# microsoft/VidTok

Measured on NVIDIA H100. Metric: frames/sec encode+decode, kl_causal_488 17x256x256, higher is better.
Workload: dtype bf16

## Files before the change

### vidtok_b200/csrc/conv_tc.cu

```cuda
#include <cuda.h>

#include <cstdio>
#include <cstdlib>
#include <cstring>
#include <string>
#include <type_traits>

#include "common.cuh"
#include "kernels.h"
#include "tc_ptx.cuh"

namespace vt {

namespace {

thread_local std::string g_tc_err;

struct TcParams {
  int B, To, Ho, Wo, Co, Ti;
  int BW, BH, BT;
  int tilesW, tilesH, tilesT;
  int num_n_tiles, BN;
  long long num_tiles;
  int kt, kh, kw, Ci, num_kc;
// ... 14 lines not shown
  int Co_real;
  int w_batched;
  int ln_mode, ln_silu;
  const float* ln_gamma;
  const float* ln_beta;
  void* out2;
  int res_mma;
  int halo, hP, a_stages;
  uint32_t halo_bytes;
  int split, a_lo, b_lo, o_lo;
  float acc_scale;
  int kparts;
  int reg_mode, reg_zc, reg_sample;
  const float* reg_noise;
  float* reg_z;
  int* reg_idx;
  double* reg_kl;
  FsqConst reg_fsq;
  uint32_t misc_off;
};

struct TcMaps {
  CUtensorMap a[4];
  CUtensorMap c;
  CUtensorMap b;
  CUtensorMap r;
  CUtensorMap e;
};

constexpr int kConsumerWarps = 8;
constexpr int kProducerWarp = kConsumerWarps;
constexpr int kThreads = (kConsumerWarps + 4) * 32;
constexpr int kABytes = 128 * 128;

using namespace tcx;

struct TileCoord {
  int b, t0, h0, w0, n0;
};
__device__ __forceinline__ TileCoord decode_tile(const TcParams& p, long long tile) {
  TileCoord c;
  const int nt = (int)(tile % p.num_n_tiles);
  long long m = tile / p.num_n_tiles;
  const int tw = (int)(m % p.tilesW); m /= p.tilesW;
  const int th = (int)(m % p.tilesH); m /= p.tilesH;
  const int tt = (int)(m % p.tilesT);
  c.b = (int)(m / p.tilesT);
  c.t0 = tt * p.BT; c.h0 = th * p.BH; c.w0 = tw * p.BW; c.n0 = nt * p.BN;
  return c;
}
__device__ __forceinline__ bool tap_time(const TcParams& p, const TileCoord& tc, int a, int& tv, bool& from_cache) {
  tv = (tc.t0 + p.to_off) * p.st + a - p.pt;
  from_cache = false;
  if (tv + p.BT <= 0) {
    if (p.t_mode == 0) return false;
    if (p.t_mode == 1) { tv = 0; return true; }
    from_cache = true;
    tv = p.cacheT + tv;
    return true;
  }
  return true;
}

__device__ __forceinline__ float quad_sum(float v) {
  v += __shfl_xor_sync(0xffffffffu, v, 1);
  v += __shfl_xor_sync(0xffffffffu, v, 2);
  return v;
}

template <int BN, bool kSplit>
__global__ void __launch_bounds__(kThreads, 1)
conv_tc_kernel(const __grid_constant__ TcMaps maps, const TcParams p) {
  extern __shared__ uint8_t smem_raw[];
  const uint32_t smem_base = (smem_u32(smem_raw) + 1023u) & ~1023u;
  uint8_t* smem_gen = smem_raw + (smem_base - smem_u32(smem_raw));
  const int warp = threadIdx.x >> 5, lane = threadIdx.x & 31;
  const uint32_t a_bytes = kABytes;
  constexpr uint32_t b_bytes = (uint32_t)BN * 128u;
  constexpr uint32_t kPl = kSplit ? 2u : 1u;
  const uint32_t stage_bytes = kPl * (p.halo ? b_bytes : a_bytes + b_bytes);
  const uint32_t win_bytes = kPl * p.halo_bytes;
  const uint32_t ring_base = smem_base + (p.halo ? (uint32_t)p.a_stages * win_bytes : 0u);
  const uint32_t bar_base = ring_base + p.stages * stage_bytes;
  auto full_bar = [&](int s) { return bar_base + 8u * s; };
  auto empty_bar = [&](int s) { return bar_base + 8u * (p.stages + s); };
  auto fullA_bar = [&](int s) { return bar_base + 8u * (2 * p.stages + s); };
  auto emptyA_bar = [&](int s) { return bar_base + 8u * (2 * p.stages + p.a_stages + s); };
  float* sbias = reinterpret_cast<float*>(smem_gen + p.misc_off);
  float* rowbuf = sbias + 2 * 768;

  if (threadIdx.x == 0) {
    for (int s = 0; s < p.stages; ++s) {
      mbar_init(full_bar(s), 1);
      mbar_init(empty_bar(s), kConsumerWarps);
    }
    for (int s = 0; s < p.a_stages; ++s) {
      mbar_init(fullA_bar(s), 1);
      mbar_init(emptyA_bar(s), kConsumerWarps);
    }
    asm volatile("fence.mbarrier_init.release.cluster;" ::: "memory");
  }
  __syncthreads();

  const int nsp = p.kh * p.kw;
  const int num_kc = p.num_kc, nstages = p.stages;
  const bool halo = p.halo != 0;
  const int res_steps = p.res_mma ? BN / 64 : 0;

  if (warp >= kProducerWarp) {
    asm volatile("setmaxnreg.dec.sync.aligned.u32 40;" ::: "memory");
    if (warp != kProducerWarp) return;
    const bool el = elect_one();
    if (el) {
      prefetch_tmap(&maps.a[0]);
      prefetch_tmap(&maps.b);
      if (p.sp == 2) { prefetch_tmap(&maps.a[1]); prefetch_tmap(&maps.a[2]); prefetch_tmap(&maps.a[3]); }
      if (p.t_mode == 2) prefetch_tmap(&maps.c);
      if (p.res_mma) { prefetch_tmap(&maps.r); prefetch_tmap(&maps.e); }
    }
    int stage = 0, sA = 0;
    uint32_t phase = 0, phA = 0;
    auto acquire = [&](uint32_t bytes) {
      mbar_wait(empty_bar(stage), phase ^ 1u);
      if (el) mbar_expect_tx(full_bar(stage), bytes);
    };
    auto advance = [&]() { if (++stage == nstages) { stage = 0; phase ^= 1u; } };
    auto load_b_planes = [&](uint32_t dst, const CUtensorMap* m, int kcol, int n, int wb_) {
      tma_load_3d(dst, m, full_bar(stage), kcol, n, wb_);
      if constexpr (kSplit) tma_load_3d(dst + b_bytes, m, full_bar(stage), p.b_lo + kcol, n, wb_);
    };
    auto load_window = [&](const CUtensorMap* m, int c0, int lo_off, int cw, int ch, int ct, int cb) {
// ... 46 lines not shown
                  const uint32_t sa = smem_base + stage * stage_bytes;
                  tma_load_5d(sa, mapA, full_bar(stage), kc * 64, cw, ch, tv, tc.b);
                  if constexpr (kSplit) tma_load_5d(sa + a_bytes, mapA, full_bar(stage), p.a_lo + kc * 64, cw, ch, tv, tc.b);
                  load_b_planes(sa + kPl * a_bytes, &maps.b, kcol + kc * 64, tc.n0, wb);
                }
                advance();
              }
            }
          }
        }
      }
      for (int g = 0; g < res_steps; ++g) {
        if (halo) {
          load_window(&maps.r, tc.n0 + g * 64, p.o_lo, tc.w0 - p.pw, tc.h0 - p.ph, tc.t0, tc.b);
          acquire(b_bytes);
          if (el) tma_load_3d(ring_base + stage * stage_bytes, &maps.e, full_bar(stage), g * 64, 0, 0);
        } else {
          acquire(kPl * a_bytes + b_bytes);
          if (el) {
            const uint32_t sa = smem_base + stage * stage_bytes;
            tma_load_5d(sa, &maps.r, full_bar(stage), tc.n0 + g * 64, tc.w0, tc.h0, tc.t0, tc.b);
            if constexpr (kSplit) tma_load_5d(sa + a_bytes, &maps.r, full_bar(stage), p.o_lo + tc.n0 + g * 64, tc.w0, tc.h0, tc.t0, tc.b);
            tma_load_3d(sa + kPl * a_bytes, &maps.e, full_bar(stage), g * 64, 0, 0);
          }
        }
        advance();
      }
    }
    return;
  }

  asm volatile("setmaxnreg.inc.sync.aligned.u32 232;" ::: "memory");
  constexpr int R = BN / 2;
  constexpr bool kSum = kSplit && BN <= 128;
  const int g = warp >> 2, wq = warp & 3;
  const bool leader = lane == 0;
  const uint32_t hi_b = desc_hi(1024u);
  const uint32_t hi_a = halo ? desc_hi((uint32_t)p.hP * 128u) : hi_b;
  const uint32_t a_row_off = halo ? (uint32_t)(8 * g) * (uint32_t)p.hP * 128u : (uint32_t)g * 64u * 128u;
  const uint32_t a_pl = halo ? p.halo_bytes : a_bytes;
  const uint32_t b_addr0 = halo ? ring_base : smem_base + kPl * a_bytes;
  float acc[R];
  float sum[kSum ? R : 1];
  int stage = 0, sA = 0, sR = 0;
  uint32_t phase = 0, phA = 0;
  int pend_stage = -1;
  bool pend_win = false;
  auto release = [&]() {
    if (leader) {
      if (pend_stage >= 0) mbar_arrive(empty_bar(pend_stage));
      if (pend_win) mbar_arrive(emptyA_bar(sR));
    }
    if (pend_win && ++sR == p.a_stages) sR = 0;
    pend_stage = -1;
    pend_win = false;
  };
  auto kstep = [&](bool a_from_stage, uint32_t a_addr, uint32_t scale, bool res, bool last_of_window) {
    mbar_wait(full_bar(stage), phase);
    if (a_from_stage) a_addr = smem_base + stage * stage_bytes + a_row_off;
    const uint32_t b_addr = b_addr0 + stage * stage_bytes;
    const uint32_t al = desc_lo(a_addr), bl = desc_lo(b_addr);
    wgmma_fence();
#pragma unroll
    for (uint32_t j = 0; j < 4u; ++j) {
      const uint64_t ah = desc(al + 2u * j, hi_a), bh = desc(bl + 2u * j, hi_b);
      wgmma_k16<BN, kSplit>(acc, ah, bh, j == 0 ? scale : 1u);
      if constexpr (kSplit) {
        wgmma_k16<BN, kSplit>(acc, desc(al + (a_pl >> 4) + 2u * j, hi_a), bh, 1u);
        if (!res) wgmma_k16<BN, kSplit>(acc, ah, desc(bl + (b_bytes >> 4) + 2u * j, hi_b), 1u);
      }
    }
    wgmma_commit();
    wgmma_wait<1>();
    release();
    pend_stage = stage;
    pend_win = last_of_window;
    if (++stage == nstages) { stage = 0; phase ^= 1u; }
  };

  const int rbase = 64 * g + 16 * wq + (lane >> 2);
  const int cq = 2 * (lane & 3);
  const bool res_direct = (p.res_mode == 1 && !p.res_mma);
  const bool store_a = (p.ln_mode != 1);
  const float inv_n = 1.0f / (float)BN;
  int last_n0 = -1;
  uint32_t cbuf = 1;

  for (long long tile = blockIdx.x; tile < p.num_tiles; tile += gridDim.x) {
    const TileCoord tc = decode_tile(p, tile);
    uint32_t G = 0xFFFFFFFFu;
    if constexpr (kSum) {
      if (p.kparts > 1) {
        uint32_t nk = 0;
        for (int a = 0; a < p.kt; ++a) {
          int tv_;
          bool fc_;
          if (tap_time(p, tc, a, tv_, fc_)) nk += (uint32_t)(nsp * num_kc);
        }
        nk += (uint32_t)res_steps;
        G = (nk + (uint32_t)p.kparts - 1u) / (uint32_t)p.kparts;
      }
#pragma unroll
      for (int i = 0; i < R; ++i) sum[i] = 0.f;
    }
    uint32_t ks = 0, accum = 0;
    auto step = [&](bool a_from_stage, uint32_t a_addr, bool res, bool last_of_window) {
      if constexpr (kSum) {
        if (ks > 0 && ks % G == 0) {
          wgmma_wait<0>();
          acc_fence(acc);
          release();
#pragma unroll
          for (int i = 0; i < R; ++i) sum[i] += acc[i];
          accum = 0;
        }
      }
      kstep(a_from_stage, a_addr, accum, res, last_of_window);
      accum = 1;
      ++ks;
    };
    for (int a = 0; a < p.kt; ++a) {
      int tv;
      bool from_cache;
      if (!tap_time(p, tc, a, tv, from_cache)) continue;
      if (halo) {
        for (int kc = 0; kc < num_kc; ++kc) {
          mbar_wait(fullA_bar(sA), phA);
          const uint32_t win = smem_base + (uint32_t)sA * win_bytes + a_row_off;
          for (int bb = 0; bb < p.kh; ++bb)
            for (int c = 0; c < p.kw; ++c)
              step(false, win + (uint32_t)(bb * p.hP + c) * 128u, false, bb == p.kh - 1 && c == p.kw - 1);
          if (++sA == p.a_stages) { sA = 0; phA ^= 1u; }
        }
      } else {
        for (int s = nsp * num_kc; s > 0; --s) step(true, 0u, false, false);
      }
    }
    for (int gr = 0; gr < res_steps; ++gr) {
      if (halo) {
        mbar_wait(fullA_bar(sA), phA);
        step(false, smem_base + (uint32_t)sA * win_bytes + a_row_off + (uint32_t)(p.ph * p.hP + p.pw) * 128u, true, true);
        if (++sA == p.a_stages) { sA = 0; phA ^= 1u; }
      } else {
        step(true, 0u, true, false);
      }
    }
    wgmma_wait<0>();
    acc_fence(acc);
    release();
    if constexpr (kSum) {
#pragma unroll
      for (int i = 0; i < R; ++i) acc[i] += sum[i];
    }

    if (tc.n0 != last_n0) {
      last_n0 = tc.n0;
      cbuf ^= 1u;
      float* b_ = sbias + cbuf * 768;
      for (int i = threadIdx.x; i < BN; i += kConsumerWarps * 32) {
        b_[i] = (p.bias && tc.n0 + i < p.Co_real) ? p.bias[tc.n0 + i] : 0.f;
        if (p.ln_mode) { const float sc = (p.ln_silu && !kSplit) ? 0.5f : 1.0f; b_[256 + i] = sc * p.ln_gamma[tc.n0 + i]; b_[512 + i] = sc * p.ln_beta[tc.n0 + i]; }
      }
      asm volatile("bar.sync 1, %0;" ::"n"(kConsumerWarps * 32) : "memory");
    }
    const float* bias_s = sbias + cbuf * 768;
    const float* gamma_s = bias_s + 256;
    const float* beta_s = bias_s + 512;

    bool valid[2];
    long long ooff[2];
    const bf16* r0[2];
    const bf16* r1[2];
    const bf16* r2[2];
    auto row_geom = [&](int row, int& t, int& h, int& w) {
      const int dw = halo ? (row & 7) : row % p.BW;
      const int dh = halo ? (row >> 3) : (row / p.BW) % p.BH;
      const int dt = halo ? 0 : row / (p.BW * p.BH);
      t = tc.t0 + dt; h = tc.h0 + dh; w = tc.w0 + dw;
      return (t < p.To) && (h < p.Ho) && (w < p.Wo);
    };
#pragma unroll
    for (int r = 0; r < 2; ++r) {
      int t, h, w;
      valid[r] = row_geom(rbase + 8 * r, t, h, w);
      ooff[r] = (long long)tc.b * p.osB + (long long)t * p.osT + (long long)h * p.osH + (long long)w * p.osW;
      r0[r] = r1[r] = r2[r] = nullptr;
      if (valid[r] && res_direct) {
        r0[r] = p.res + (long long)tc.b * p.rsB + (long long)t * p.rsT + (long long)h * p.rsH + (long long)w * p.rsW + tc.n0;
      } else if (valid[r] && p.res_mode == 3) {
        const long long sp = (long long)tc.b * p.rsB + (long long)h * p.rsH + (long long)w * p.rsW + tc.n0;
        const int ta = 2 * t - 1 + p.res_pool_off, tb = ta + 1, tcn = ta + 2;
        if (ta >= 0) r0[r] = p.res + sp + (long long)ta * p.rsT;
        else if (p.res_t_mode == 1) r0[r] = p.res + sp;
        else if (p.res_t_mode == 2) r0[r] = p.res_cache + (((long long)tc.b * p.Ho + h) * p.Wo + w) * (long long)p.Co * (kSplit ? 2 : 1) + tc.n0;
        if (tb < p.resT) r1[r] = p.res + sp + (long long)tb * p.rsT;
        if (tcn < p.resT) r2[r] = p.res + sp + (long long)tcn * p.rsT;
      }
    }
    auto res_pair = [&](const bf16* rp, int c, float& x0, float& x1) {
      const uint32_t hw = *reinterpret_cast<const uint32_t*>(rp + c);
      if constexpr (kSplit) {
        const uint32_t lw = *reinterpret_cast<const uint32_t*>(rp + p.o_lo + c);
        x0 = f16_lo(hw) + f16_lo(lw);
        x1 = f16_hi(hw) + f16_hi(lw);
      } else {
        x0 = bf16_lo(hw);
        x1 = bf16_hi(hw);
      }
    };
#pragma unroll
    for (int j = 0; j < BN / 8; ++j) {
      const int c = 8 * j + cq;
#pragma unroll
      for (int e = 0; e < 4; ++e) {
        float f = kSplit ? fmaf(acc[4 * j + e], p.acc_scale, bias_s[c + (e & 1)]) : acc[4 * j + e] + bias_s[c + (e & 1)];
        if (p.rb != 1.0f) f *= p.rb;
        acc[4 * j + e] = f;
      }
#pragma unroll
      for (int r = 0; r < 2; ++r) {
        if (!valid[r]) continue;
        if (res_direct) {
          float x0, x1;
          res_pair(r0[r], c, x0, x1);
          acc[4 * j + 2 * r] = fmaf(p.ra, x0, acc[4 * j + 2 * r]);
          acc[4 * j + 2 * r + 1] = fmaf(p.ra, x1, acc[4 * j + 2 * r + 1]);
        } else if (p.res_mode == 3) {
          float s0 = 0.f, s1 = 0.f, x0, x1;
          if (r0[r]) { res_pair(r0[r], c, x0, x1); s0 += x0; s1 += x1; }
          if (r1[r]) { res_pair(r1[r], c, x0, x1); s0 += x0; s1 += x1; }
          if (r2[r]) { res_pair(r2[r], c, x0, x1); s0 += x0; s1 += x1; }
          const float s3 = p.ra * (1.0f / 3.0f);
          acc[4 * j + 2 * r] = fmaf(s3, s0, acc[4 * j + 2 * r]);
          acc[4 * j + 2 * r + 1] = fmaf(s3, s1, acc[4 * j + 2 * r + 1]);
        }
      }
    }

    if (p.out_f32) {
      if (p.out) {
#pragma unroll
        for (int r = 0; r < 2; ++r) {
          if (!valid[r]) continue;
          float* of = reinterpret_cast<float*>(p.out) + ooff[r];
#pragma unroll
          for (int j = 0; j < BN / 8; ++j)
#pragma unroll
            for (int e = 0; e < 2; ++e) {
              const int n = tc.n0 + 8 * j + cq + e;
              if (n < p.Co_real) of[(long long)n * p.osC] = acc[4 * j + 2 * r + e];
            }
        }
      }
      if (p.reg_mode) {
        if constexpr (BN == 32) {
#pragma unroll
          for (int j = 0; j < 4; ++j)
#pragma unroll
            for (int e = 0; e < 4; ++e) rowbuf[(rbase + 8 * (e >> 1)) * 33 + 8 * j + cq + (e & 1)] = acc[4 * j + e];
          asm volatile("bar.sync 2, %0;" ::"n"(kConsumerWarps * 32) : "memory");
          if (threadIdx.x < 128) {
            const int row = threadIdx.x;
            float f[32];
#pragma unroll
            for (int c = 0; c < 32; ++c) f[c] = rowbuf[row * 33 + c];
            int t, h, w;
            const bool ok = row_geom(row, t, h, w);
            const long long plane = p.osC;
            const long long pos = (long long)t * p.osT + (long long)h * p.osH + (long long)w * p.osW;
            if (p.reg_mode == 1) {
              float part = 0.f;
              auto kl_row = [&](auto ZC) {
                constexpr int zc = decltype(ZC)::value;
                const long long zb = (long long)tc.b * zc * plane + pos;
#pragma unroll
                for (int c = 0; c < zc; ++c) {
                  float zv;
                  part += kl_sample_one(f[c], f[zc + c], p.reg_sample ? p.reg_noise[zb + c * plane] : 0.f, p.reg_sample, zv);
                  p.reg_z[zb + c * plane] = zv;
                }
              };
              if (ok) {
                if (p.reg_zc == 4) kl_row(std::integral_constant<int, 4>());
                else if (p.reg_zc == 8) kl_row(std::integral_constant<int, 8>());
                else kl_row(std::integral_constant<int, 16>());
              }
              double dsum = (double)part;
#pragma unroll
              for (int o = 16; o > 0; o >>= 1) dsum += __shfl_xor_sync(0xffffffffu, dsum, o);
              if (lane == 0) atomicAdd(p.reg_kl, dsum);
            } else if (ok) {
              const long long zb = (long long)tc.b * p.reg_zc * plane + pos;
              float idx = 0.f;
#pragma unroll
              for (int c = 0; c < VT_MAX_FSQ; ++c)
                if (c < p.reg_zc) p.reg_z[zb + c * plane] = fsq_code(p.reg_fsq, c, f[c], idx);
              if (p.reg_idx) p.reg_idx[(long long)tc.b * plane + pos] = (int)idx;
            }
          }
          asm volatile("bar.sync 2, %0;" ::"n"(kConsumerWarps * 32) : "memory");
        }
      }
      continue;
    }

    auto put = [&](void* optr, int r, int c, float y0, float y1) {
      bf16* o = reinterpret_cast<bf16*>(optr) + ooff[r] + tc.n0 + c;
      if constexpr (kSplit) {
        const uint32_t hw = pack_f16x2(y0, y1);
        *reinterpret_cast<uint32_t*>(o) = hw;
        *reinterpret_cast<uint32_t*>(o + p.o_lo) = pack_f16x2(y0 - f16_lo(hw), y1 - f16_hi(hw));
      } else {
        *reinterpret_cast<uint32_t*>(o) = pack_bf16x2(y0, y1);
      }
    };
    if constexpr (kSplit) {
      if (store_a) {
#pragma unroll
        for (int r = 0; r < 2; ++r)
          if (valid[r])
#pragma unroll
            for (int j = 0; j < BN / 8; ++j) put(p.out, r, 8 * j + cq, acc[4 * j + 2 * r], acc[4 * j + 2 * r + 1]);
      }
      if (p.ln_mode) {
        void* nout = p.ln_mode == 1 ? p.out : p.out2;
#pragma unroll
        for (int r = 0; r < 2; ++r) {
          float s = 0.f;
#pragma unroll
          for (int j = 0; j < BN / 8; ++j) s += acc[4 * j + 2 * r] + acc[4 * j + 2 * r + 1];
          const float mean = quad_sum(s) * inv_n;
          float q = 0.f;
#pragma unroll
          for (int j = 0; j < BN / 8; ++j) {
            const float d0 = acc[4 * j + 2 * r] - mean, d1 = acc[4 * j + 2 * r + 1] - mean;
            q = fmaf(d0, d0, q);
            q = fmaf(d1, d1, q);
          }
          const float rstd = 1.0f / sqrtf(quad_sum(q) * inv_n + 1e-6f);
          if (!valid[r]) continue;
#pragma unroll
          for (int j = 0; j < BN / 8; ++j) {
            const int c = 8 * j + cq;
            float y0 = (acc[4 * j + 2 * r] - mean) * rstd * gamma_s[c] + beta_s[c];
            float y1 = (acc[4 * j + 2 * r + 1] - mean) * rstd * gamma_s[c + 1] + beta_s[c + 1];
            if (p.ln_silu) { y0 = silu_tc(y0); y1 = silu_tc(y1); }
            put(nout, r, c, y0, y1);
          }
        }
      }
    } else {
#pragma unroll
      for (int r = 0; r < 2; ++r) {
        float s = 0.f, q = 0.f;
#pragma unroll
        for (int j = 0; j < BN / 8; ++j) {
          const float f0 = acc[4 * j + 2 * r], f1 = acc[4 * j + 2 * r + 1];
          s += f0 + f1;
          q = fmaf(f0, f0, q);
          q = fmaf(f1, f1, q);
          const uint32_t kp = pack_bf16x2(f0, f1);
          if (store_a && valid[r]) *reinterpret_cast<uint32_t*>(reinterpret_cast<bf16*>(p.out) + ooff[r] + tc.n0 + 8 * j + cq) = kp;
          acc[4 * j + 2 * r] = bf16_lo(kp);
          acc[4 * j + 2 * r + 1] = bf16_hi(kp);
        }
        if (!p.ln_mode) continue;
        const float mean = quad_sum(s) * inv_n;
        float var = fmaf(-mean, mean, quad_sum(q) * inv_n);
        var = var < 0.f ? 0.f : var;
        const float rstd = rsqrtf(var + 1e-6f);
        const float nmr = -mean * rstd;
        if (!valid[r]) continue;
        void* nout = p.ln_mode == 1 ? p.out : p.out2;
#pragma unroll
        for (int j = 0; j < BN / 8; ++j) {
          const int c = 8 * j + cq;
          float y0 = fmaf(fmaf(acc[4 * j + 2 * r], rstd, nmr), gamma_s[c], beta_s[c]);
          float y1 = fmaf(fmaf(acc[4 * j + 2 * r + 1], rstd, nmr), gamma_s[c + 1], beta_s[c + 1]);
          if (p.ln_silu) {
            y0 = fmaf(y0, tanh_approx(y0), y0);
            y1 = fmaf(y1, tanh_approx(y1), y1);
          }
          put(nout, r, c, y0, y1);
        }
      }
    }
  }
}

__global__ void fill_identity_kernel(bf16* e, int f16, float value) {
  const int r = blockIdx.x, c = threadIdx.x;
  if (f16) reinterpret_cast<__half*>(e)[r * 256 + c] = __float2half_rn(r == c ? value : 0.0f);
  else e[r * 256 + c] = __float2bfloat16_rn(r == c ? value : 0.0f);
}

typedef CUresult (*EncodeTiledFn)(CUtensorMap*, CUtensorMapDataType, cuuint32_t, void*, const cuuint64_t*,
                                  const cuuint64_t*, const cuuint32_t*, const cuuint32_t*, CUtensorMapInterleave,
                                  CUtensorMapSwizzle, CUtensorMapL2promotion, CUtensorMapFloatOOBfill);
EncodeTiledFn get_encode() {
  static EncodeTiledFn fn = nullptr;
  static bool tried = false;
  if (!tried) {
    tried = true;
    void* p = nullptr;
    cudaDriverEntryPointQueryResult q;
    if (cudaGetDriverEntryPoint("cuTensorMapEncodeTiled", &p, cudaEnableDefault, &q) == cudaSuccess &&
        q == cudaDriverEntryPointSuccess)
      fn = (EncodeTiledFn)p;
  }
  return fn;
}

constexpr int kMaxDev = 64;
int device_num_sms() {
  static int sms[kMaxDev] = {0};
  int dev = 0;
// ... 102 lines not shown
  EncodeTiledFn enc = get_encode();
  if (!enc) { g_tc_err = "cuTensorMapEncodeTiled unavailable"; return cudaErrorNotSupported; }
  const bool split = p.split != 0;
  const int cw = split ? 2 : 1;
  const bool out_bf16 = tout != DT_F32;
  if (split != (tout == DT_SPLIT) && tout != DT_F32) { g_tc_err = "split activations need a split (or fp32) output"; return cudaErrorInvalidValue; }
  TcParams t;
  memset(&t, 0, sizeof(t));
  const int Co_pad = (p.Co + 31) / 32 * 32;
  const int num_sms = device_num_sms();
  static int halo_env = -1;
  if (halo_env < 0) { const char* e = getenv("VT_TC_HALO"); halo_env = e ? atoi(e) : 1; }
  size_t smem = 0;
  auto plan = [&](bool allow_halo, int bn_cap) -> int {
    t.halo = 0; t.hP = 0; t.a_stages = 0; t.halo_bytes = 0;
    t.BN = choose_bn(Co_pad);
    if (bn_cap && t.BN > bn_cap) t.BN = bn_cap;
    if (!choose_tile(p, 128, t.BW, t.BH, t.BT)) { g_tc_err = "no tile shape"; return -1; }
    const bool geom = p.sh == 1 && p.sw == 1 && p.kh * p.kw > 1 && p.kh <= 3 && p.kw <= 3 && p.Ho == p.Hi && p.Wo == p.Wi &&
                      w_batches <= 1 && p.Wo % 8 == 0 && p.Ho % 16 == 0;
    if (allow_halo && halo_env && geom) {
      t.halo = 1;
      t.BW = 8; t.BH = 16; t.BT = 1;
      t.hP = 16;
      t.halo_bytes = (uint32_t)((16 + p.kh - 1) * t.hP * 128);
      t.a_stages = 2;
    }
    t.tilesW = (p.Wo + t.BW - 1) / t.BW; t.tilesH = (p.Ho + t.BH - 1) / t.BH; t.tilesT = (p.To + t.BT - 1) / t.BT;
    t.num_n_tiles = Co_pad / t.BN;
    t.num_tiles = (long long)p.B * t.tilesT * t.tilesH * t.tilesW * t.num_n_tiles;
    const size_t stage_bytes = (size_t)cw * ((t.halo ? 0 : (size_t)kABytes) + (size_t)t.BN * 128);
    const size_t budget = 225 * 1024;
    const size_t a_ring = (size_t)t.a_stages * t.halo_bytes * cw;
    const size_t misc = 2 * 768 * 4 + ((reg && reg->mode) ? 128 * 33 * 4 : 0);
    const size_t fixed = 1024  + misc + 16;
    if (budget < fixed + a_ring + 2 * (stage_bytes + 16)) return 1;
    int stages = (int)((budget - fixed - a_ring) / (stage_bytes + 16));
    if (stages > 8) stages = 8;
    {
      static int cap = -1;
      if (cap < 0) { const char* e = getenv("VT_TC_STAGES"); cap = e ? atoi(e) : 0; }
      if (cap >= 2 && stages > cap) stages = cap;
    }
    t.stages = stages;
    const size_t bars = 8 * (2 * (size_t)stages + 2 * (size_t)t.a_stages);
    t.misc_off = (uint32_t)((a_ring + stages * stage_bytes + bars + 15) & ~(size_t)15);
    smem = 1024 + t.misc_off + misc;
    t.kparts = 1;
    const int nk_ = p.kt * p.kh * p.kw * (p.Ci / 64);
    if (split && t.BN <= 128 && nk_ >= 16) t.kparts = nk_ >= 64 ? 8 : 4;
    return 0;
  };
  {
    const bool need_row = ln && ln->mode;
    const int nk = p.kt * p.kh * p.kw * (p.Ci / 64);
    const int bn_pref = (split && !need_row && w_batches <= 1) ? (nk >= 128 ? 64 : (nk >= 16 ? 128 : 0)) : 0;
    int rc = plan(true, bn_pref);
    if (rc == 1) rc = plan(false, bn_pref);
    if (rc == 1 && !need_row) rc = plan(false, 128);
    if (rc == 1) g_tc_err = "not enough shared memory for 2 stages";
    if (rc != 0) return cudaErrorInvalidValue;
  }
  t.split = split ? 1 : 0; t.a_lo = p.Ci; t.b_lo = Kpad; t.o_lo = p.Co;
  t.acc_scale = (split && p.acc_scale != 0.f) ? p.acc_scale : 1.0f;
  t.B = p.B; t.To = p.To; t.Ho = p.Ho; t.Wo = p.Wo; t.Co = p.Co; t.Ti = p.Ti;
  t.kt = p.kt; t.kh = p.kh; t.kw = p.kw; t.Ci = p.Ci; t.num_kc = p.Ci / 64;
  t.st = p.st; t.pt = p.pt; t.ph = p.ph; t.pw = p.pw; t.to_off = p.to_off; t.sp = p.sh;
// ... 138 lines not shown
```

### vidtok_b200/csrc/tc_ptx.cuh

```cuda
#pragma once
#include <cuda.h>
#include <cuda_bf16.h>
#include <cuda_fp16.h>
#include <stdint.h>

namespace vt {
namespace tcx {
__device__ __forceinline__ uint32_t smem_u32(const void* p) { return (uint32_t)__cvta_generic_to_shared(p); }

__device__ __forceinline__ void mbar_init(uint32_t bar, uint32_t count) {
  asm volatile("mbarrier.init.shared::cta.b64 [%0], %1;" ::"r"(bar), "r"(count) : "memory");
}
__device__ __forceinline__ void mbar_expect_tx(uint32_t bar, uint32_t bytes) {
  asm volatile("mbarrier.arrive.expect_tx.shared::cta.b64 _, [%0], %1;" ::"r"(bar), "r"(bytes) : "memory");
}
__device__ __forceinline__ void mbar_arrive(uint32_t bar) {
  asm volatile("mbarrier.arrive.shared::cta.b64 _, [%0];" ::"r"(bar) : "memory");
}
__device__ __forceinline__ bool mbar_try_wait(uint32_t bar, uint32_t parity) {
  uint32_t ok;
  asm volatile(
      "{\n\t"
      ".reg .pred p;\n\t"
      "mbarrier.try_wait.parity.shared::cta.b64 p, [%1], %2;\n\t"
      "selp.u32 %0, 1, 0, p;\n\t"
      "}"
      : "=r"(ok)
      : "r"(bar), "r"(parity)
      : "memory");
  return ok != 0;
}
__device__ __forceinline__ void mbar_wait(uint32_t bar, uint32_t parity) {
  if (mbar_try_wait(bar, parity)) return;
  const long long t0 = clock64();
  while (!mbar_try_wait(bar, parity)) {
    if (clock64() - t0 > 8000000000LL) __trap();
  }
}
__device__ __forceinline__ void tma_load_5d(uint32_t dst, const CUtensorMap* map, uint32_t bar, int c0, int c1, int c2,
                                            int c3, int c4) {
  asm volatile(
      "cp.async.bulk.tensor.5d.shared::cluster.global.mbarrier::complete_tx::bytes [%0], [%1, {%3, %4, %5, %6, %7}], [%2];"
      ::"r"(dst), "l"(map), "r"(bar), "r"(c0), "r"(c1), "r"(c2), "r"(c3), "r"(c4)
      : "memory");
}
__device__ __forceinline__ void tma_load_3d(uint32_t dst, const CUtensorMap* map, uint32_t bar, int c0, int c1, int c2) {
  asm volatile(
      "cp.async.bulk.tensor.3d.shared::cluster.global.mbarrier::complete_tx::bytes [%0], [%1, {%3, %4, %5}], [%2];"
      ::"r"(dst), "l"(map), "r"(bar), "r"(c0), "r"(c1), "r"(c2)
      : "memory");
}
__device__ __forceinline__ void fence_async_smem() { asm volatile("fence.proxy.async.shared::cta;" ::: "memory"); }
__device__ __forceinline__ void prefetch_tmap(const CUtensorMap* map) {
  asm volatile("prefetch.tensormap [%0];" ::"l"(map) : "memory");
}
__device__ __forceinline__ bool elect_one() {
  uint32_t pred;
  asm volatile(
      "{\n\t"
      ".reg .pred P1;\n\t"
      "elect.sync _|P1, 0xffffffff;\n\t"
      "selp.u32 %0, 1, 0, P1;\n\t"
      "}"
      : "=r"(pred));
  return pred != 0;
}

__device__ __forceinline__ void wgmma_fence() { asm volatile("wgmma.fence.sync.aligned;" ::: "memory"); }
__device__ __forceinline__ void wgmma_commit() { asm volatile("wgmma.commit_group.sync.aligned;" ::: "memory"); }
template <int kPending>
__device__ __forceinline__ void wgmma_wait() { asm volatile("wgmma.wait_group.sync.aligned %0;" ::"n"(kPending) : "memory"); }
template <int R>
__device__ __forceinline__ void acc_fence(float (&d)[R]) {
#pragma unroll
  for (int i = 0; i < R; ++i) asm volatile("" : "+f"(d[i])::"memory");
}

__device__ __forceinline__ uint32_t desc_lo(uint32_t saddr) { return ((saddr & 0x3FFFFu) >> 4) | (1u << 16); }
__device__ __forceinline__ uint32_t desc_hi(uint32_t sbo) { return (sbo >> 4) | (1u << 30); }
__device__ __forceinline__ uint64_t desc(uint32_t lo, uint32_t hi) { return ((uint64_t)hi << 32) | lo; }

__device__ __forceinline__ void wgmma_32_bf16(float (&d)[16], uint64_t da, uint64_t db, uint32_t scale_d) {
  asm volatile(
      "{\n\t.reg .pred p;\n\t"
      "setp.ne.b32 p, %18, 0;\n\t"
// ... 205 lines not shown
```

Measured before the change: 301.5.

## Add ping-pong consumer warpgroup scheduling for non-split BN64/128 conv tiles

For non-split convolutions with BN 64 or 128, the two consumer warpgroups now alternate whole tiles instead of splitting each tile's M rows. Each warpgroup computes the full 128-row tile into two accumulator halves. Named barriers hand over MMA turns so one group's epilogue overlaps the other group's mainloop, and the skipping group advances its stage and phase counters to stay in step with the producer. This doubles accumulator registers per thread and adds per-group bias buffers and barrier handoff logic. Pipeline-phase accounting is fragile and could hang if it does not match what the producer actually issues.

```diff
diff --git a/vidtok_b200/csrc/conv_tc.cu b/vidtok_b200/csrc/conv_tc.cu
--- a/vidtok_b200/csrc/conv_tc.cu
+++ b/vidtok_b200/csrc/conv_tc.cu
@@ -70,6 +70,9 @@
 constexpr int kProducerWarp = kConsumerWarps;
 constexpr int kThreads = (kConsumerWarps + 4) * 32;
 constexpr int kABytes = 128 * 128;
+constexpr uint32_t kBarTurn = 3, kBarBias = 5;
+
+__host__ __device__ constexpr bool ping_pong(int BN, bool split) { return !split && (BN == 64 || BN == 128); }
 
 using namespace tcx;
 
@@ -98,6 +101,15 @@
     return true;
   }
   return true;
+}
+__device__ __forceinline__ int tile_taps(const TcParams& p, const TileCoord& tc) {
+  int n = 0;
+  for (int a = 0; a < p.kt; ++a) {
+    int tv;
+    bool from_cache;
+    if (tap_time(p, tc, a, tv, from_cache)) ++n;
+  }
+  return n;
 }
 
 __device__ __forceinline__ float quad_sum(float v) {
@@ -124,17 +136,19 @@
   auto empty_bar = [&](int s) { return bar_base + 8u * (p.stages + s); };
   auto fullA_bar = [&](int s) { return bar_base + 8u * (2 * p.stages + s); };
   auto emptyA_bar = [&](int s) { return bar_base + 8u * (2 * p.stages + p.a_stages + s); };
+  constexpr bool kPingPong = ping_pong(BN, kSplit);
   float* sbias = reinterpret_cast<float*>(smem_gen + p.misc_off);
   float* rowbuf = sbias + 2 * 768;
 
   if (threadIdx.x == 0) {
+    constexpr uint32_t readers = kPingPong ? kConsumerWarps / 2 : kConsumerWarps;
     for (int s = 0; s < p.stages; ++s) {
       mbar_init(full_bar(s), 1);
-      mbar_init(empty_bar(s), kConsumerWarps);
+      mbar_init(empty_bar(s), readers);
     }
     for (int s = 0; s < p.a_stages; ++s) {
       mbar_init(fullA_bar(s), 1);
-      mbar_init(emptyA_bar(s), kConsumerWarps);
+      mbar_init(emptyA_bar(s), readers);
     }
     asm volatile("fence.mbarrier_init.release.cluster;" ::: "memory");
   }
@@ -247,15 +261,17 @@
 
   asm volatile("setmaxnreg.inc.sync.aligned.u32 232;" ::: "memory");
   constexpr int R = BN / 2;
+  constexpr int kHalves = kPingPong ? 2 : 1;
   constexpr bool kSum = kSplit && BN <= 128;
   const int g = warp >> 2, wq = warp & 3;
   const bool leader = lane == 0;
   const uint32_t hi_b = desc_hi(1024u);
   const uint32_t hi_a = halo ? desc_hi((uint32_t)p.hP * 128u) : hi_b;
-  const uint32_t a_row_off = halo ? (uint32_t)(8 * g) * (uint32_t)p.hP * 128u : (uint32_t)g * 64u * 128u;
+  const uint32_t a_half = halo ? 8u * (uint32_t)p.hP * 128u : 64u * 128u;
+  const uint32_t a_row_off = kPingPong ? 0u : (uint32_t)g * a_half;
   const uint32_t a_pl = halo ? p.halo_bytes : a_bytes;
   const uint32_t b_addr0 = halo ? ring_base : smem_base + kPl * a_bytes;
-  float acc[R];
+  float acc[kHalves][R];
   float sum[kSum ? R : 1];
   int stage = 0, sA = 0, sR = 0;
   uint32_t phase = 0, phA = 0;
@@ -279,10 +295,11 @@
 #pragma unroll
     for (uint32_t j = 0; j < 4u; ++j) {
       const uint64_t ah = desc(al + 2u * j, hi_a), bh = desc(bl + 2u * j, hi_b);
-      wgmma_k16<BN, kSplit>(acc, ah, bh, j == 0 ? scale : 1u);
+      wgmma_k16<BN, kSplit>(acc[0], ah, bh, j == 0 ? scale : 1u);
+      if constexpr (kPingPong) wgmma_k16<BN, kSplit>(acc[1], desc(al + (a_half >> 4) + 2u * j, hi_a), bh, j == 0 ? scale : 1u);
       if constexpr (kSplit) {
-        wgmma_k16<BN, kSplit>(acc, desc(al + (a_pl >> 4) + 2u * j, hi_a), bh, 1u);
-        if (!res) wgmma_k16<BN, kSplit>(acc, ah, desc(bl + (b_bytes >> 4) + 2u * j, hi_b), 1u);
+        wgmma_k16<BN, kSplit>(acc[0], desc(al + (a_pl >> 4) + 2u * j, hi_a), bh, 1u);
+        if (!res) wgmma_k16<BN, kSplit>(acc[0], ah, desc(bl + (b_bytes >> 4) + 2u * j, hi_b), 1u);
       }
     }
     wgmma_commit();
@@ -293,7 +310,7 @@
     if (++stage == nstages) { stage = 0; phase ^= 1u; }
   };
 
-  const int rbase = 64 * g + 16 * wq + (lane >> 2);
+  const int rbase = (kPingPong ? 0 : 64 * g) + 16 * wq + (lane >> 2);
   const int cq = 2 * (lane & 3);
   const bool res_direct = (p.res_mode == 1 && !p.res_mma);
   const bool store_a = (p.ln_mode != 1);
@@ -301,18 +318,30 @@
   int last_n0 = -1;
   uint32_t cbuf = 1;
 
-  for (long long tile = blockIdx.x; tile < p.num_tiles; tile += gridDim.x) {
+  int owner = 0;
+  for (long long tile = blockIdx.x; tile < p.num_tiles; tile += gridDim.x, owner ^= 1) {
     const TileCoord tc = decode_tile(p, tile);
+    if constexpr (kPingPong) {
+      if (owner != g) {
+        const int taps = tile_taps(p, tc);
+        stage += taps * nsp * num_kc + res_steps;
+        if ((stage / nstages) & 1) phase ^= 1u;
+        stage %= nstages;
+        if (halo) {
+          const int nw = taps * num_kc + res_steps;
+          sA += nw;
+          if ((sA / p.a_stages) & 1) phA ^= 1u;
+          sA %= p.a_stages;
+          sR = (sR + nw) % p.a_stages;
+        }
+        continue;
+      }
+      if (tile != blockIdx.x) named_bar_sync(kBarTurn + g, kConsumerWarps * 32);
+    }
     uint32_t G = 0xFFFFFFFFu;
     if constexpr (kSum) {
       if (p.kparts > 1) {
-        uint32_t nk = 0;
-        for (int a = 0; a < p.kt; ++a) {
-          int tv_;
-          bool fc_;
-          if (tap_time(p, tc, a, tv_, fc_)) nk += (uint32_t)(nsp * num_kc);
-        }
-        nk += (uint32_t)res_steps;
+        const uint32_t nk = (uint32_t)(tile_taps(p, tc) * nsp * num_kc + res_steps);
         G = (nk + (uint32_t)p.kparts - 1u) / (uint32_t)p.kparts;
       }
 #pragma unroll
@@ -323,10 +352,10 @@
       if constexpr (kSum) {
         if (ks > 0 && ks % G == 0) {
           wgmma_wait<0>();
-          acc_fence(acc);
+          acc_fence(acc[0]);
           release();
 #pragma unroll
-          for (int i = 0; i < R; ++i) sum[i] += acc[i];
+          for (int i = 0; i < R; ++i) sum[i] += acc[0][i];
           accum = 0;
         }
       }
@@ -360,243 +389,260 @@
         step(true, 0u, true, false);
       }
     }
+    if constexpr (kPingPong) {
+      if (tile + gridDim.x < p.num_tiles) named_bar_arrive(kBarTurn + (g ^ 1), kConsumerWarps * 32);
+    }
     wgmma_wait<0>();
-    acc_fence(acc);
+#pragma unroll
+    for (int hf = 0; hf < kHalves; ++hf) acc_fence(acc[hf]);
     release();
     if constexpr (kSum) {
 #pragma unroll
-      for (int i = 0; i < R; ++i) acc[i] += sum[i];
+      for (int i = 0; i < R; ++i) acc[0][i] += sum[i];
     }
 
     if (tc.n0 != last_n0) {
       last_n0 = tc.n0;
       cbuf ^= 1u;
-      float* b_ = sbias + cbuf * 768;
-      for (int i = threadIdx.x; i < BN; i += kConsumerWarps * 32) {
+      constexpr int nthr = kPingPong ? 128 : kConsumerWarps * 32;
+      float* b_ = sbias + ((kPingPong ? 2 * g : 0) + cbuf) * 768;
+      for (int i = threadIdx.x % nthr; i < BN; i += nthr) {
         b_[i] = (p.bias && tc.n0 + i < p.Co_real) ? p.bias[tc.n0 + i] : 0.f;
         if (p.ln_mode) { const float sc = (p.ln_silu && !kSplit) ? 0.5f : 1.0f; b_[256 + i] = sc * p.ln_gamma[tc.n0 + i]; b_[512 + i] = sc * p.ln_beta[tc.n0 + i]; }
       }
-      asm volatile("bar.sync 1, %0;" ::"n"(kConsumerWarps * 32) : "memory");
-    }
-    const float* bias_s = sbias + cbuf * 768;
+      named_bar_sync(kPingPong ? kBarBias + g : 1u, nthr);
+    }
+    const float* bias_s = sbias + ((kPingPong ? 2 * g : 0) + cbuf) * 768;
     const float* gamma_s = bias_s + 256;
     const float* beta_s = bias_s + 512;
 
-    bool valid[2];
-    long long ooff[2];
-    const bf16* r0[2];
-    const bf16* r1[2];
-    const bf16* r2[2];
-    auto row_geom = [&](int row, int& t, int& h, int& w) {
-      const int dw = halo ? (row & 7) : row % p.BW;
-      const int dh = halo ? (row >> 3) : (row / p.BW) % p.BH;
-      const int dt = halo ? 0 : row / (p.BW * p.BH);
-      t = tc.t0 + dt; h = tc.h0 + dh; w = tc.w0 + dw;
-      return (t < p.To) && (h < p.Ho) && (w < p.Wo);
-    };
-#pragma unroll
-    for (int r = 0; r < 2; ++r) {
-      int t, h, w;
-      valid[r] = row_geom(rbase + 8 * r, t, h, w);
-      ooff[r] = (long long)tc.b * p.osB + (long long)t * p.osT + (long long)h * p.osH + (long long)w * p.osW;
-      r0[r] = r1[r] = r2[r] = nullptr;
-      if (valid[r] && res_direct) {
-        r0[r] = p.res + (long long)tc.b * p.rsB + (long long)t * p.rsT + (long long)h * p.rsH + (long long)w * p.rsW + tc.n0;
-      } else if (valid[r] && p.res_mode == 3) {
-        const long long sp = (long long)tc.b * p.rsB + (long long)h * p.rsH + (long long)w * p.rsW + tc.n0;
-        const int ta = 2 * t - 1 + p.res_pool_off, tb = ta + 1, tcn = ta + 2;
-        if (ta >= 0) r0[r] = p.res + sp + (long long)ta * p.rsT;
-        else if (p.res_t_mode == 1) r0[r] = p.res + sp;
-        else if (p.res_t_mode == 2) r0[r] = p.res_cache + (((long long)tc.b * p.Ho + h) * p.Wo + w) * (long long)p.Co * (kSplit ? 2 : 1) + tc.n0;
-        if (tb < p.resT) r1[r] = p.res + sp + (long long)tb * p.rsT;
-        if (tcn < p.resT) r2[r] = p.res + sp + (long long)tcn * p.rsT;
-      }
-    }
-    auto res_pair = [&](const bf16* rp, int c, float& x0, float& x1) {
-      const uint32_t hw = *reinterpret_cast<const uint32_t*>(rp + c);
-      if constexpr (kSplit) {
-        const uint32_t lw = *reinterpret_cast<const uint32_t*>(rp + p.o_lo + c);
-        x0 = f16_lo(hw) + f16_lo(lw);
-        x1 = f16_hi(hw) + f16_hi(lw);
-      } else {
-        x0 = bf16_lo(hw);
-        x1 = bf16_hi(hw);
-      }
-    };
-#pragma unroll
-    for (int j = 0; j < BN / 8; ++j) {
-      const int c = 8 * j + cq;
-#pragma unroll
-      for (int e = 0; e < 4; ++e) {
-        float f = kSplit ? fmaf(acc[4 * j + e], p.acc_scale, bias_s[c + (e & 1)]) : acc[4 * j + e] + bias_s[c + (e & 1)];
-        if (p.rb != 1.0f) f *= p.rb;
-        acc[4 * j + e] = f;
-      }
+#pragma unroll
+    for (int hf = 0; hf < kHalves; ++hf) {
+      float (&acc_h)[R] = acc[hf];
+      int row0 = rbase + 64 * hf;
+      asm volatile("" : "+r"(row0));
+      bool valid[2];
+      long long ooff[2];
+      auto row_geom = [&](int row, int& t, int& h, int& w) {
+        const int dw = halo ? (row & 7) : row % p.BW;
+        const int dh = halo ? (row >> 3) : (row / p.BW) % p.BH;
+        const int dt = halo ? 0 : row / (p.BW * p.BH);
+        t = tc.t0 + dt; h = tc.h0 + dh; w = tc.w0 + dw;
+        return (t < p.To) && (h < p.Ho) && (w < p.Wo);
+      };
 #pragma unroll
       for (int r = 0; r < 2; ++r) {
-        if (!valid[r]) continue;
-        if (res_direct) {
-          float x0, x1;
-          res_pair(r0[r], c, x0, x1);
-          acc[4 * j + 2 * r] = fmaf(p.ra, x0, acc[4 * j + 2 * r]);
-          acc[4 * j + 2 * r + 1] = fmaf(p.ra, x1, acc[4 * j + 2 * r + 1]);
-        } else if (p.res_mode == 3) {
-          float s0 = 0.f, s1 = 0.f, x0, x1;
-          if (r0[r]) { res_pair(r0[r], c, x0, x1); s0 += x0; s1 += x1; }
-          if (r1[r]) { res_pair(r1[r], c, x0, x1); s0 += x0; s1 += x1; }
-          if (r2[r]) { res_pair(r2[r], c, x0, x1); s0 += x0; s1 += x1; }
-          const float s3 = p.ra * (1.0f / 3.0f);
-          acc[4 * j + 2 * r] = fmaf(s3, s0, acc[4 * j + 2 * r]);
-          acc[4 * j + 2 * r + 1] = fmaf(s3, s1, acc[4 * j + 2 * r + 1]);
-        }
-      }
-    }
-
-    if (p.out_f32) {
-      if (p.out) {
+        int t, h, w;
+        valid[r] = row_geom(row0 + 8 * r, t, h, w);
+        ooff[r] = (long long)tc.b * p.osB + (long long)t * p.osT + (long long)h * p.osH + (long long)w * p.osW;
+      }
+      auto res_pair = [&](const bf16* rp, int c, float& x0, float& x1) {
+        const uint32_t hw = *reinterpret_cast<const uint32_t*>(rp + c);
+        if constexpr (kSplit) {
+          const uint32_t lw = *reinterpret_cast<const uint32_t*>(rp + p.o_lo + c);
+          x0 = f16_lo(hw) + f16_lo(lw);
+          x1 = f16_hi(hw) + f16_hi(lw);
+        } else {
+          x0 = bf16_lo(hw);
+          x1 = bf16_hi(hw);
+        }
+      };
+#pragma unroll
+      for (int j = 0; j < BN / 8; ++j) {
+        const int c = 8 * j + cq;
+#pragma unroll
+        for (int e = 0; e < 4; ++e) {
+          float f = kSplit ? fmaf(acc_h[4 * j + e], p.acc_scale, bias_s[c + (e & 1)]) : acc_h[4 * j + e] + bias_s[c + (e & 1)];
+          if (p.rb != 1.0f) f *= p.rb;
+          acc_h[4 * j + e] = f;
+        }
+      }
+      if (res_direct || p.res_mode == 3) {
 #pragma unroll
         for (int r = 0; r < 2; ++r) {
-          if (!valid[r]) continue;
-          float* of = reinterpret_cast<float*>(p.out) + ooff[r];
-#pragma unroll
-          for (int j = 0; j < BN / 8; ++j)
-#pragma unroll
-            for (int e = 0; e < 2; ++e) {
-              const int n = tc.n0 + 8 * j + cq + e;
-              if (n < p.Co_real) of[(long long)n * p.osC] = acc[4 * j + 2 * r + e];
-            }
-        }
-      }
-      if (p.reg_mode) {
-        if constexpr (BN == 32) {
-#pragma unroll
-          for (int j = 0; j < 4; ++j)
-#pragma unroll
-            for (int e = 0; e < 4; ++e) rowbuf[(rbase + 8 * (e >> 1)) * 33 + 8 * j + cq + (e & 1)] = acc[4 * j + e];
-          asm volatile("bar.sync 2, %0;" ::"n"(kConsumerWarps * 32) : "memory");
-          if (threadIdx.x < 128) {
-            const int row = threadIdx.x;
-            float f[32];
-#pragma unroll
-            for (int c = 0; c < 32; ++c) f[c] = rowbuf[row * 33 + c];
-            int t, h, w;
-            const bool ok = row_geom(row, t, h, w);
-            const long long plane = p.osC;
-            const long long pos = (long long)t * p.osT + (long long)h * p.osH + (long long)w * p.osW;
-            if (p.reg_mode == 1) {
-              float part = 0.f;
-              auto kl_row = [&](auto ZC) {
-                constexpr int zc = decltype(ZC)::value;
-                const long long zb = (long long)tc.b * zc * plane + pos;
-#pragma unroll
-                for (int c = 0; c < zc; ++c) {
-                  float zv;
-                  part += kl_sample_one(f[c], f[zc + c], p.reg_sample ? p.reg_noise[zb + c * plane] : 0.f, p.reg_sample, zv);
-                  p.reg_z[zb + c * plane] = zv;
-                }
-              };
-              if (ok) {
-                if (p.reg_zc == 4) kl_row(std::integral_constant<int, 4>());
-                else if (p.reg_zc == 8) kl_row(std::integral_constant<int, 8>());
-                else kl_row(std::integral_constant<int, 16>());
-              }
-              double dsum = (double)part;
-#pragma unroll
-              for (int o = 16; o > 0; o >>= 1) dsum += __shfl_xor_sync(0xffffffffu, dsum, o);
-              if (lane == 0) atomicAdd(p.reg_kl, dsum);
-            } else if (ok) {
-              const long long zb = (long long)tc.b * p.reg_zc * plane + pos;
-              float idx = 0.f;
-#pragma unroll
-              for (int c = 0; c < VT_MAX_FSQ; ++c)
-                if (c < p.reg_zc) p.reg_z[zb + c * plane] = fsq_code(p.reg_fsq, c, f[c], idx);
-              if (p.reg_idx) p.reg_idx[(long long)tc.b * plane + pos] = (int)idx;
+          int t, h, w;
+          if (!row_geom(row0 + 8 * r, t, h, w)) continue;
+          const bf16* r0 = nullptr;
+          const bf16* r1 = nullptr;
+          const bf16* r2 = nullptr;
+          if (res_direct) {
+            r0 = p.res + (long long)tc.b * p.rsB + (long long)t * p.rsT + (long long)h * p.rsH + (long long)w * p.rsW + tc.n0;
+          } else {
+            const long long sp = (long long)tc.b * p.rsB + (long long)h * p.rsH + (long long)w * p.rsW + tc.n0;
+            const int ta = 2 * t - 1 + p.res_pool_off, tb = ta + 1, tcn = ta + 2;
+            if (ta >= 0) r0 = p.res + sp + (long long)ta * p.rsT;
+            else if (p.res_t_mode == 1) r0 = p.res + sp;
+            else if (p.res_t_mode == 2) r0 = p.res_cache + (((long long)tc.b * p.Ho + h) * p.Wo + w) * (long long)p.Co * (kSplit ? 2 : 1) + tc.n0;
+            if (tb < p.resT) r1 = p.res + sp + (long long)tb * p.rsT;
+            if (tcn < p.resT) r2 = p.res + sp + (long long)tcn * p.rsT;
+          }
+#pragma unroll
+          for (int j = 0; j < BN / 8; ++j) {
+            const int c = 8 * j + cq;
+            if (res_direct) {
+              float x0, x1;
+              res_pair(r0, c, x0, x1);
+              acc_h[4 * j + 2 * r] = fmaf(p.ra, x0, acc_h[4 * j + 2 * r]);
+              acc_h[4 * j + 2 * r + 1] = fmaf(p.ra, x1, acc_h[4 * j + 2 * r + 1]);
+            } else {
+              float s0 = 0.f, s1 = 0.f, x0, x1;
+              if (r0) { res_pair(r0, c, x0, x1); s0 += x0; s1 += x1; }
+              if (r1) { res_pair(r1, c, x0, x1); s0 += x0; s1 += x1; }
+              if (r2) { res_pair(r2, c, x0, x1); s0 += x0; s1 += x1; }
+              const float s3 = p.ra * (1.0f / 3.0f);
+              acc_h[4 * j + 2 * r] = fmaf(s3, s0, acc_h[4 * j + 2 * r]);
+              acc_h[4 * j + 2 * r + 1] = fmaf(s3, s1, acc_h[4 * j + 2 * r + 1]);
             }
           }
-          asm volatile("bar.sync 2, %0;" ::"n"(kConsumerWarps * 32) : "memory");
-        }
-      }
-      continue;
-    }
-
-    auto put = [&](void* optr, int r, int c, float y0, float y1) {
-      bf16* o = reinterpret_cast<bf16*>(optr) + ooff[r] + tc.n0 + c;
+        }
+      }
+
+      if (p.out_f32) {
+        if (p.out) {
+#pragma unroll
+          for (int r = 0; r < 2; ++r) {
+            if (!valid[r]) continue;
+            float* of = reinterpret_cast<float*>(p.out) + ooff[r];
+#pragma unroll
+            for (int j = 0; j < BN / 8; ++j)
+#pragma unroll
+              for (int e = 0; e < 2; ++e) {
+                const int n = tc.n0 + 8 * j + cq + e;
+                if (n < p.Co_real) of[(long long)n * p.osC] = acc_h[4 * j + 2 * r + e];
+              }
+          }
+        }
+        if (p.reg_mode) {
+          if constexpr (BN == 32) {
+#pragma unroll
+            for (int j = 0; j < 4; ++j)
+#pragma unroll
+              for (int e = 0; e < 4; ++e) rowbuf[(rbase + 8 * (e >> 1)) * 33 + 8 * j + cq + (e & 1)] = acc_h[4 * j + e];
+            asm volatile("bar.sync 2, %0;" ::"n"(kConsumerWarps * 32) : "memory");
+            if (threadIdx.x < 128) {
+              const int row = threadIdx.x;
+              float f[32];
+#pragma unroll
+              for (int c = 0; c < 32; ++c) f[c] = rowbuf[row * 33 + c];
+              int t, h, w;
+              const bool ok = row_geom(row, t, h, w);
+              const long long plane = p.osC;
+              const long long pos = (long long)t * p.osT + (long long)h * p.osH + (long long)w * p.osW;
+              if (p.reg_mode == 1) {
+                float part = 0.f;
+                auto kl_row = [&](auto ZC) {
+                  constexpr int zc = decltype(ZC)::value;
+                  const long long zb = (long long)tc.b * zc * plane + pos;
+#pragma unroll
+                  for (int c = 0; c < zc; ++c) {
+                    float zv;
+                    part += kl_sample_one(f[c], f[zc + c], p.reg_sample ? p.reg_noise[zb + c * plane] : 0.f, p.reg_sample, zv);
+                    p.reg_z[zb + c * plane] = zv;
+                  }
+                };
+                if (ok) {
+                  if (p.reg_zc == 4) kl_row(std::integral_constant<int, 4>());
+                  else if (p.reg_zc == 8) kl_row(std::integral_constant<int, 8>());
+                  else kl_row(std::integral_constant<int, 16>());
+                }
+                double dsum = (double)part;
+#pragma unroll
+                for (int o = 16; o > 0; o >>= 1) dsum += __shfl_xor_sync(0xffffffffu, dsum, o);
+                if (lane == 0) atomicAdd(p.reg_kl, dsum);
+              } else if (ok) {
+                const long long zb = (long long)tc.b * p.reg_zc * plane + pos;
+                float idx = 0.f;
+#pragma unroll
+                for (int c = 0; c < VT_MAX_FSQ; ++c)
+                  if (c < p.reg_zc) p.reg_z[zb + c * plane] = fsq_code(p.reg_fsq, c, f[c], idx);
+                if (p.reg_idx) p.reg_idx[(long long)tc.b * plane + pos] = (int)idx;
+              }
+            }
+            asm volatile("bar.sync 2, %0;" ::"n"(kConsumerWarps * 32) : "memory");
+          }
+        }
+        continue;
+      }
+
+      auto put = [&](void* optr, int r, int c, float y0, float y1) {
+        bf16* o = reinterpret_cast<bf16*>(optr) + ooff[r] + tc.n0 + c;
+        if constexpr (kSplit) {
+          const uint32_t hw = pack_f16x2(y0, y1);
+          *reinterpret_cast<uint32_t*>(o) = hw;
+          *reinterpret_cast<uint32_t*>(o + p.o_lo) = pack_f16x2(y0 - f16_lo(hw), y1 - f16_hi(hw));
+        } else {
+          *reinterpret_cast<uint32_t*>(o) = pack_bf16x2(y0, y1);
+        }
+      };
       if constexpr (kSplit) {
-        const uint32_t hw = pack_f16x2(y0, y1);
-        *reinterpret_cast<uint32_t*>(o) = hw;
-        *reinterpret_cast<uint32_t*>(o + p.o_lo) = pack_f16x2(y0 - f16_lo(hw), y1 - f16_hi(hw));
+        if (store_a) {
+#pragma unroll
+          for (int r = 0; r < 2; ++r)
+            if (valid[r])
+#pragma unroll
+              for (int j = 0; j < BN / 8; ++j) put(p.out, r, 8 * j + cq, acc_h[4 * j + 2 * r], acc_h[4 * j + 2 * r + 1]);
+        }
+        if (p.ln_mode) {
+          void* nout = p.ln_mode == 1 ? p.out : p.out2;
+#pragma unroll
+          for (int r = 0; r < 2; ++r) {
+            float s = 0.f;
+#pragma unroll
+            for (int j = 0; j < BN / 8; ++j) s += acc_h[4 * j + 2 * r] + acc_h[4 * j + 2 * r + 1];
+            const float mean = quad_sum(s) * inv_n;
+            float q = 0.f;
+#pragma unroll
+            for (int j = 0; j < BN / 8; ++j) {
+              const float d0 = acc_h[4 * j + 2 * r] - mean, d1 = acc_h[4 * j + 2 * r + 1] - mean;
+              q = fmaf(d0, d0, q);
+              q = fmaf(d1, d1, q);
+            }
+            const float rstd = 1.0f / sqrtf(quad_sum(q) * inv_n + 1e-6f);
+            if (!valid[r]) continue;
+#pragma unroll
+            for (int j = 0; j < BN / 8; ++j) {
+              const int c = 8 * j + cq;
+              float y0 = (acc_h[4 * j + 2 * r] - mean) * rstd * gamma_s[c] + beta_s[c];
+              float y1 = (acc_h[4 * j + 2 * r + 1] - mean) * rstd * gamma_s[c + 1] + beta_s[c + 1];
+              if (p.ln_silu) { y0 = silu_tc(y0); y1 = silu_tc(y1); }
+              put(nout, r, c, y0, y1);
+            }
+          }
+        }
       } else {
-        *reinterpret_cast<uint32_t*>(o) = pack_bf16x2(y0, y1);
-      }
-    };
-    if constexpr (kSplit) {
-      if (store_a) {
-#pragma unroll
-        for (int r = 0; r < 2; ++r)
-          if (valid[r])
-#pragma unroll
-            for (int j = 0; j < BN / 8; ++j) put(p.out, r, 8 * j + cq, acc[4 * j + 2 * r], acc[4 * j + 2 * r + 1]);
-      }
-      if (p.ln_mode) {
-        void* nout = p.ln_mode == 1 ? p.out : p.out2;
 #pragma unroll
         for (int r = 0; r < 2; ++r) {
-          float s = 0.f;
-#pragma unroll
-          for (int j = 0; j < BN / 8; ++j) s += acc[4 * j + 2 * r] + acc[4 * j + 2 * r + 1];
+          float s = 0.f, q = 0.f;
+#pragma unroll
+          for (int j = 0; j < BN / 8; ++j) {
+            const float f0 = acc_h[4 * j + 2 * r], f1 = acc_h[4 * j + 2 * r + 1];
+            s += f0 + f1;
+            q = fmaf(f0, f0, q);
+            q = fmaf(f1, f1, q);
+            const uint32_t kp = pack_bf16x2(f0, f1);
+            if (store_a && valid[r]) *reinterpret_cast<uint32_t*>(reinterpret_cast<bf16*>(p.out) + ooff[r] + tc.n0 + 8 * j + cq) = kp;
+            acc_h[4 * j + 2 * r] = bf16_lo(kp);
+            acc_h[4 * j + 2 * r + 1] = bf16_hi(kp);
+          }
+          if (!p.ln_mode) continue;
           const float mean = quad_sum(s) * inv_n;
-          float q = 0.f;
-#pragma unroll
-          for (int j = 0; j < BN / 8; ++j) {
-            const float d0 = acc[4 * j + 2 * r] - mean, d1 = acc[4 * j + 2 * r + 1] - mean;
-            q = fmaf(d0, d0, q);
-            q = fmaf(d1, d1, q);
-          }
-          const float rstd = 1.0f / sqrtf(quad_sum(q) * inv_n + 1e-6f);
+          float var = fmaf(-mean, mean, quad_sum(q) * inv_n);
+          var = var < 0.f ? 0.f : var;
+          const float rstd = rsqrtf(var + 1e-6f);
+          const float nmr = -mean * rstd;
           if (!valid[r]) continue;
+          void* nout = p.ln_mode == 1 ? p.out : p.out2;
 #pragma unroll
           for (int j = 0; j < BN / 8; ++j) {
             const int c = 8 * j + cq;
-            float y0 = (acc[4 * j + 2 * r] - mean) * rstd * gamma_s[c] + beta_s[c];
-            float y1 = (acc[4 * j + 2 * r + 1] - mean) * rstd * gamma_s[c + 1] + beta_s[c + 1];
-            if (p.ln_silu) { y0 = silu_tc(y0); y1 = silu_tc(y1); }
+            float y0 = fmaf(fmaf(acc_h[4 * j + 2 * r], rstd, nmr), gamma_s[c], beta_s[c]);
+            float y1 = fmaf(fmaf(acc_h[4 * j + 2 * r + 1], rstd, nmr), gamma_s[c + 1], beta_s[c + 1]);
+            if (p.ln_silu) {
+              y0 = fmaf(y0, tanh_approx(y0), y0);
+              y1 = fmaf(y1, tanh_approx(y1), y1);
+            }
             put(nout, r, c, y0, y1);
           }
-        }
-      }
-    } else {
-#pragma unroll
-      for (int r = 0; r < 2; ++r) {
-        float s = 0.f, q = 0.f;
-#pragma unroll
-        for (int j = 0; j < BN / 8; ++j) {
-          const float f0 = acc[4 * j + 2 * r], f1 = acc[4 * j + 2 * r + 1];
-          s += f0 + f1;
-          q = fmaf(f0, f0, q);
-          q = fmaf(f1, f1, q);
-          const uint32_t kp = pack_bf16x2(f0, f1);
-          if (store_a && valid[r]) *reinterpret_cast<uint32_t*>(reinterpret_cast<bf16*>(p.out) + ooff[r] + tc.n0 + 8 * j + cq) = kp;
-          acc[4 * j + 2 * r] = bf16_lo(kp);
-          acc[4 * j + 2 * r + 1] = bf16_hi(kp);
-        }
-        if (!p.ln_mode) continue;
-        const float mean = quad_sum(s) * inv_n;
-        float var = fmaf(-mean, mean, quad_sum(q) * inv_n);
-        var = var < 0.f ? 0.f : var;
-        const float rstd = rsqrtf(var + 1e-6f);
-        const float nmr = -mean * rstd;
-        if (!valid[r]) continue;
-        void* nout = p.ln_mode == 1 ? p.out : p.out2;
-#pragma unroll
-        for (int j = 0; j < BN / 8; ++j) {
-          const int c = 8 * j + cq;
-          float y0 = fmaf(fmaf(acc[4 * j + 2 * r], rstd, nmr), gamma_s[c], beta_s[c]);
-          float y1 = fmaf(fmaf(acc[4 * j + 2 * r + 1], rstd, nmr), gamma_s[c + 1], beta_s[c + 1]);
-          if (p.ln_silu) {
-            y0 = fmaf(y0, tanh_approx(y0), y0);
-            y1 = fmaf(y1, tanh_approx(y1), y1);
-          }
-          put(nout, r, c, y0, y1);
         }
       }
     }
@@ -765,7 +811,7 @@
     const size_t stage_bytes = (size_t)cw * ((t.halo ? 0 : (size_t)kABytes) + (size_t)t.BN * 128);
     const size_t budget = 225 * 1024;
     const size_t a_ring = (size_t)t.a_stages * t.halo_bytes * cw;
-    const size_t misc = 2 * 768 * 4 + ((reg && reg->mode) ? 128 * 33 * 4 : 0);
+    const size_t misc = (ping_pong(t.BN, split) ? 4 : 2) * 768 * 4 + ((reg && reg->mode) ? 128 * 33 * 4 : 0);
     const size_t fixed = 1024  + misc + 16;
     if (budget < fixed + a_ring + 2 * (stage_bytes + 16)) return 1;
     int stages = (int)((budget - fixed - a_ring) / (stage_bytes + 16));
diff --git a/vidtok_b200/csrc/tc_ptx.cuh b/vidtok_b200/csrc/tc_ptx.cuh
--- a/vidtok_b200/csrc/tc_ptx.cuh
+++ b/vidtok_b200/csrc/tc_ptx.cuh
@@ -51,6 +51,12 @@
       : "memory");
 }
 __device__ __forceinline__ void fence_async_smem() { asm volatile("fence.proxy.async.shared::cta;" ::: "memory"); }
+__device__ __forceinline__ void named_bar_sync(uint32_t id, uint32_t threads) {
+  asm volatile("bar.sync %0, %1;" ::"r"(id), "r"(threads) : "memory");
+}
+__device__ __forceinline__ void named_bar_arrive(uint32_t id, uint32_t threads) {
+  asm volatile("bar.arrive %0, %1;" ::"r"(id), "r"(threads) : "memory");
+}
 __device__ __forceinline__ void prefetch_tmap(const CUtensorMap* map) {
   asm volatile("prefetch.tensormap [%0];" ::"l"(map) : "memory");
 }
```

Result: faster. 333.4, median of 6 (+10.6%).
